# StorjOld/heartbeat

Hardware: AMD Instinct MI355X
Metric: GiB/s file bytes tagged (Swizzle encode, device-resident) at 1/2/4/8 GPUs (higher is better)
Workload: dtype u32

## Files before the change

heartbeat_amd/csrc/hb_args.hpp:

```cpp
#pragma once
#include "hb_lane.hpp"
#include "hb_digest_cache.hpp"

extern thread_local bool hb_load_only;

#ifndef HB_ENGINE_WG
#define HB_ENGINE_WG 1024
#endif
#define HB_ENGINE_WG_PER_CU 1
#ifndef HB_QUEUE_CHUNK
#define HB_QUEUE_CHUNK 256
#endif
#define HB_MAX_TRIES 2048u
#define HB_QSLOT 4
#define HB_SLOT_RETRY 7

#ifndef HB_RETRY_DIGEST
#define HB_RETRY_DIGEST 1
#endif
struct HbRetry {
    u64 blk;
    u32 flags;
    u32 pad_;
    u32 sr[4];
    u32 part[8];
#if HB_RETRY_DIGEST
    u32 dig[8];
#endif
};

#define HB_MFMA_MAX_S 2048u
#if defined(HB_MFMA_TOEPLITZ)
#define HB_MFMA_NT 2
#else
#define HB_MFMA_NT 1
#endif

template <int NL>
struct EncodeArgs {
    PrfParams<NL> prf;
    ModP<NL> mod;
    const unsigned char *data;
    u64 len;
    u64 nblocks;
    u64 block_base;
    unsigned char *tags;
    const u32 *alpha_mont;
    const u32 *t0;
// ... 225 lines not shown
```

heartbeat_amd/csrc/hb_kernels.hpp:

```cpp
#pragma once
#include <hip/hip_runtime.h>
#include "hb_args.hpp"
#include "hb_mac_src.hpp"

#define HB_LDS_WORDS (HB_TAB_BYTES / 4)

__device__ __forceinline__ void hb_fill_lds(u32 *lds, const u32 *t0) {
    for (u32 g = threadIdx.x; g < HB_LDS_WORDS / 4; g += blockDim.x) {
        const u32 off = g * 16u;
        const u32 e = (off >> 8) & 0xffu, t = ((off >> 16) << 1) | ((off >> 7) & 1u);
        u32 v = t0[e];
        if (t) v = (v << (8 * t)) | (v >> (32 - 8 * t));
        reinterpret_cast<uint4 *>(lds)[g] = make_uint4(v, v, v, v);
    }
    __syncthreads();
}

__device__ __forceinline__ LaneTab hb_lane_tab(const u32 *lds) {
    const u32 r4 = (threadIdx.x & 31u) * 4u;
    return LaneTab{(const char *)lds, {r4, 128u + r4, 0x10000u | r4, 0x10000u | (128u + r4)}};
}

__device__ __forceinline__ u32 hb_lane_id() { return threadIdx.x & 63u; }

// ... 22 lines not shown
        u64 base2 = 0, got2 = 0;
        if (avail < need && !exhausted) {
            u64 b = 0;
            if (hb_lane_id() == 0) b = atomicAdd(counter, (unsigned long long)chunk);
            b = hb_bcast64(b);
            if (b >= njobs) {
                exhausted = true;
            } else {
                base2 = b;
                got2 = njobs - b < chunk ? njobs - b : chunk;
            }
        }
        bool ok = false;
        if (want) {
            if ((u64)rank < avail) {
                job = next + rank;
                ok = true;
            } else if ((u64)rank - avail < got2) {
                job = base2 + ((u64)rank - avail);
                ok = true;
            }
        }
        if ((u64)need <= avail) {
            next += need;
        } else {
            const u64 used2 = (u64)need - avail < got2 ? (u64)need - avail : got2;
            next = base2 + used2;
            end = base2 + got2;
        }
        return ok;
    }
};

template <int MODE>
__device__ __forceinline__ void hb_prf_digest(u64 x, u32 dig[8]) {
    if (MODE != 0) hb_sha256_le32((u32)x, dig);
    else hb_sha256_decimal(x, dig);
}

template <int MODE, class H>
__device__ __forceinline__ auto hb_job_digest(const H &h, u64 job, u32 dig[8], int)
    -> decltype(h.digest(job, dig), void()) {
    if (!h.digest(job, dig)) hb_prf_digest<MODE>(h.x_of(job), dig);
}
template <int MODE, class H>
__device__ __forceinline__ void hb_job_digest(const H &h, u64 job, u32 dig[8], long) {
    hb_prf_digest<MODE>(h.x_of(job), dig);
}

template <class H>
__device__ __forceinline__ auto hb_resumed_tries(const H &, int) -> decltype(H::kResumedTries, u32()) {
    return H::kResumedTries;
}
template <class H>
__device__ __forceinline__ u32 hb_resumed_tries(const H &, long) { return 0u; }

template <int NL, int NR, class H, int MODE = 0>
__device__ __forceinline__ void hb_engine(H &h, const LaneTab &L, const PrfParams<NL> &P,
                                          u64 njobs, unsigned long long *queue, u64 chunk = HB_QUEUE_CHUNK) {
    HbPool pool{0, 0, njobs, queue, false, chunk};
    u64 job = 0;
    bool active = pool.take(__ballot(1), true, job);
    u32 dig[8], sr[4] = {0, 0, 0, 0}, out[NL];
    if (active) {
        h.init(job, sr);
        hb_job_digest<MODE>(h, job, dig, 0);
    }
    const u32 resumed = hb_resumed_tries(h, 0);
    u32 tries = 0, job_tries = resumed, failed = 0;
    while (__ballot(active)) {
        u32 ok;
        if constexpr (MODE == 1) ok = hb_cxx_try<NL, NR>(L, P, sr, dig, out);
        else if constexpr (MODE == 2) ok = hb_cxx_try_bytes<NL, NR>(L, P, sr, dig, out, job_tries);
        else ok = hb_prf_try<NL, NR>(L, P, sr, dig, out);
        tries += active ? 1u : 0u;
        job_tries += 1u;
        if (MODE != 0 && job_tries >= HB_CXX_MAX_TRIES) ok = 1;
        const bool acc = active && ok;
        if (acc) h.accept(job, out);
        const bool give_up = active && !ok && job_tries >= HB_MAX_TRIES;
        failed += give_up ? 1u : 0u;
        const bool next = acc || give_up;
        const u64 m = __ballot(next);
        if (m) {
            u64 nj = 0;
            const bool got = pool.take(m, next, nj);
            if (next) {
                active = got;
                job = nj;
                job_tries = resumed;
                if (got) {
                    h.init(job, sr);
                    hb_job_digest<MODE>(h, job, dig, 0);
                }
            }
        }
    }
    for (int off = 32; off > 0; off >>= 1) {
        tries += __shfl_xor(tries, off);
        failed += __shfl_xor(failed, off);
    }
    if (hb_lane_id() == 0 && tries) atomicAdd(queue + 1, (unsigned long long)tries);
    if (hb_lane_id() == 0 && failed) atomicAdd(queue + 2, (unsigned long long)failed);
}

#define HB_QP(a, b, c, d) ((a) | ((b) << 2) | ((c) << 4) | ((d) << 6))

template <int CTRL>
__device__ __forceinline__ u32 hb_qdpp(u32 x) {
    return (u32)__builtin_amdgcn_mov_dpp((int)x, CTRL, 0xf, 0xf, false);
}
__device__ __forceinline__ u64 hb_qbcast64(u64 v) {
    const u32 lo = hb_qdpp<HB_QP(0, 0, 0, 0)>((u32)v), hi = hb_qdpp<HB_QP(0, 0, 0, 0)>((u32)(v >> 32));
    return ((u64)hi << 32) | lo;
}

struct QuadLane {
    LaneTab L;
    u32 lbq;
// ... 68 lines not shown
        if (nw == 0) word &= (P.topmask << (24 - sh)) | (0xffffffu >> sh);
        HB_UNROLL
        for (int t = NL - 1; t > 0; --t) out[t] = hb_alignbit(out[t], out[t - 1], sh);
        out[0] = hb_alignbit(out[0], word << sh, sh);
    }
    u32 borrow = 0;
    HB_UNROLL
    for (int t = 0; t < NL; ++t) {
        u64 d = (u64)out[t] - (u64)P.R[t] - (u64)borrow;
        borrow = (u32)(d >> 63);
    }
    return borrow;
}

template <int NL, int NR, class H>
__device__ __forceinline__ void hb_engine_quad(H &h, const LaneTab &L, const PrfParams<NL> &P, u64 njobs,
                                               unsigned long long *queue, u64 chunk, u64 first = ~0ull,
                                               u64 end = ~0ull) {
    const QuadLane Q = hb_quad_lane(L);
    const u32 q = hb_lane_id() & 3u;
    const bool lead = q == 0;
    u32 rkq[NR + 1];
    HB_UNROLL
    for (int r = 0; r <= NR; ++r) {
        const u32 k0 = __builtin_amdgcn_readfirstlane(P.rk[4 * r]), k1 = __builtin_amdgcn_readfirstlane(P.rk[4 * r + 1]);
        const u32 k2 = __builtin_amdgcn_readfirstlane(P.rk[4 * r + 2]), k3 = __builtin_amdgcn_readfirstlane(P.rk[4 * r + 3]);
        rkq[r] = q == 0 ? k0 : q == 1 ? k1 : q == 2 ? k2 : k3;
    }
    u64 stop = njobs - first < 16 ? njobs : first + 16;
    if (stop > end) stop = end;
    HbPool pool = first == ~0ull ? HbPool{0, 0, njobs, queue, false, chunk}
                                 : HbPool{first, stop, njobs, queue, true, chunk};
    u64 job = 0;
    bool active = pool.take(__ballot(lead), lead, job);
    job = hb_qbcast64(job);
    active = hb_qdpp<HB_QP(0, 0, 0, 0)>(active ? 1u : 0u) != 0;
    u32 dig[8], s = 0, out[NL];
    if (active) hb_job_digest<0>(h, job, dig, 0);
    u32 tries = 0, job_tries = 0, failed = 0;
    while (__ballot(active)) {
        const u32 ok = hb_quad_prf_try<NL, NR>(Q, rkq, P, s, dig, out);
        tries += active && lead ? 1u : 0u;
        job_tries += 1u;
        const bool acc = active && ok;
        if (acc && lead) h.accept(job, out);
        const bool give_up = active && !ok && job_tries >= HB_MAX_TRIES;
        failed += give_up && lead ? 1u : 0u;
        if (give_up && lead) h.fail(job);
        const bool next = acc || give_up;
        const u64 m = __ballot(next && lead);
        if (m) {
            u64 nj = 0;
            bool got = pool.take(m, next && lead, nj);
            nj = hb_qbcast64(nj);
            got = hb_qdpp<HB_QP(0, 0, 0, 0)>(got ? 1u : 0u) != 0;
            if (next) {
                active = got;
                job = nj;
                job_tries = 0;
                if (got) {
                    s = 0;
                    hb_job_digest<0>(h, job, dig, 0);
                }
            }
        }
    }
    for (int off = 32; off > 0; off >>= 1) {
        tries += __shfl_xor(tries, off);
        failed += __shfl_xor(failed, off);
    }
    if (hb_lane_id() == 0 && tries) atomicAdd(queue + 1, (unsigned long long)tries);
    if (hb_lane_id() == 0 && failed) atomicAdd(queue + 2, (unsigned long long)failed);
}

#ifndef HB_RETRY_QUAD_TAIL
#define HB_RETRY_QUAD_TAIL 1
#endif
template <int NL, int NR, class H>
__device__ __forceinline__ void hb_engine_tail(H &h, const LaneTab &L, const PrfParams<NL> &P, u64 njobs,
                                               unsigned long long *queue, u64 chunk) {
    HbPool pool{0, 0, njobs, queue, false, chunk};
    u64 job = 0;
    bool active = pool.take(__ballot(1), true, job);
    u32 dig[8], sr[4] = {0, 0, 0, 0}, out[NL];
    if (active) {
        h.init(job, sr);
        hb_job_digest<0>(h, job, dig, 0);
    }
    const u32 resumed = hb_resumed_tries(h, 0);
    u32 tries = 0, job_tries = resumed, failed = 0;
    u64 am;
    while ((am = __ballot(active)) != 0) {
        if (pool.exhausted && pool.next >= pool.end && __popcll(am) <= 16) break;
        const u32 ok = hb_prf_try<NL, NR>(L, P, sr, dig, out);
        tries += active ? 1u : 0u;
        job_tries += 1u;
        const bool acc = active && ok;
        if (acc) h.accept(job, out);
        const bool give_up = active && !ok && job_tries >= HB_MAX_TRIES;
        failed += give_up ? 1u : 0u;
        const bool next = acc || give_up;
        const u64 m = __ballot(next);
        if (m) {
            u64 nj = 0;
            const bool got = pool.take(m, next, nj);
            if (next) {
                active = got;
                job = nj;
                job_tries = resumed;
                if (got) {
                    h.init(job, sr);
                    hb_job_digest<0>(h, job, dig, 0);
                }
            }
        }
    }
    if (am) {
        const u32 lane = hb_lane_id(), r = lane >> 2, q = lane & 3u;
        const bool qa = r < (u32)__popcll(am);
        u64 mm = am;
        for (u32 k = 0; k < r && mm; ++k) mm &= mm - 1;
        const int src = mm ? __builtin_ctzll(mm) : 0;
        const u64 qjob = ((u64)(u32)__shfl((int)(u32)(job >> 32), src) << 32) | (u32)__shfl((int)(u32)job, src);
        u32 qdig[8];
        HB_UNROLL
        for (int t = 0; t < 8; ++t) qdig[t] = (u32)__shfl((int)dig[t], src);
        const u32 w0 = (u32)__shfl((int)sr[0], src), w1 = (u32)__shfl((int)sr[1], src);
        const u32 w2 = (u32)__shfl((int)sr[2], src), w3 = (u32)__shfl((int)sr[3], src);
        u32 s = q == 0 ? w0 : q == 1 ? w1 : q == 2 ? w2 : w3;
        u32 jt = (u32)__shfl((int)job_tries, src);
        const QuadLane Q = hb_quad_lane(L);
        u32 rkq[NR + 1];
        HB_UNROLL
        for (int rr = 0; rr <= NR; ++rr) {
            const u32 k0 = __builtin_amdgcn_readfirstlane(P.rk[4 * rr]), k1 = __builtin_amdgcn_readfirstlane(P.rk[4 * rr + 1]);
            const u32 k2 = __builtin_amdgcn_readfirstlane(P.rk[4 * rr + 2]), k3 = __builtin_amdgcn_readfirstlane(P.rk[4 * rr + 3]);
            rkq[rr] = q == 0 ? k0 : q == 1 ? k1 : q == 2 ? k2 : k3;
        }
// ... 419 lines not shown
    v[NL] = T[NL] + (u32)c;
    hb_reduce_small<NL>(v, M, out);
}
#endif

template <int NL>
__device__ __forceinline__ uint4 *hb_dig_entry(const EncodeArgs<NL> &A, u64 blk) {
    return reinterpret_cast<uint4 *>(A.dig_tab + (A.block_base + blk - A.dig_lo) * 8);
}

template <int NL>
__device__ __forceinline__ void hb_dig_load(const EncodeArgs<NL> &A, u64 blk, u32 dig[8]) {
    const uint4 *e = hb_dig_entry<NL>(A, blk);
    const uint4 a = e[0], b = e[1];
    dig[0] = a.x; dig[1] = a.y; dig[2] = a.z; dig[3] = a.w;
    dig[4] = b.x; dig[5] = b.y; dig[6] = b.z; dig[7] = b.w;
}

template <int NL, bool DLOAD>
__device__ __forceinline__ void hb_first_digest(const EncodeArgs<NL> &A, u64 job, bool act, u32 dig[8]) {
    if constexpr (DLOAD) {
        hb_dig_load<NL>(A, job, dig);
        return;
    }
    hb_sha256_decimal(A.block_base + job, dig);
    if (A.dig_mode == HB_DIG_STORE && act) {
        uint4 *e = hb_dig_entry<NL>(A, job);
        e[0] = make_uint4(dig[0], dig[1], dig[2], dig[3]);
        e[1] = make_uint4(dig[4], dig[5], dig[6], dig[7]);
    }
}

template <int NL>
__device__ __forceinline__ void hb_list_early(const EncodeArgs<NL> &A, u64 job, u64 mask, const u32 dig[8],
                                              u64 &base) {
#if HB_RETRY_DIGEST
    u64 b = 0;
    if (hb_lane_id() == 0) b = atomicAdd(A.retry_count, (unsigned long long)__popcll(mask));
    base = hb_bcast64(b);
    if ((mask >> hb_lane_id()) & 1ull) {
        const u64 slot = base + hb_mbcnt(mask);
        if (slot < A.retry_cap) {
            HbRetry *e = A.retry + slot;
            *reinterpret_cast<uint4 *>(e) = make_uint4((u32)job, (u32)(job >> 32), 1u, 0u);
            *reinterpret_cast<uint4 *>(e->dig) = make_uint4(dig[0], dig[1], dig[2], dig[3]);
            *reinterpret_cast<uint4 *>(e->dig + 4) = make_uint4(dig[4], dig[5], dig[6], dig[7]);
        }
    }
#endif
}

template <int NL, int NR, int ALIGN, class H>
__device__ __forceinline__ void hb_first_finish(const EncodeArgs<NL> &A, const LaneTab &L, H &h, u64 job,
                                                bool active, u32 ok, u32 sr[4], u32 out[NL], u32 &tries,
                                                u32 &failed, u32 *T, bool tmine, u64 pre_base, u64 pre_mask) {
    tries += active ? 1u : 0u;
    const bool rejected = active && !ok;
    const bool pre = (pre_mask >> hb_lane_id()) & 1ull;
    const u64 rej = __ballot(rejected && !pre);
    bool listed = false;
    HbRetry *e = nullptr;
    if (pre) {
        const u64 slot = pre_base + hb_mbcnt(pre_mask);
        if (slot < A.retry_cap) {
            listed = true;
            e = A.retry + slot;
        }
    }
    if (rej) {
        u64 base = 0;
        if (hb_lane_id() == 0) base = atomicAdd(A.retry_count, (unsigned long long)__popcll(rej));
        base = hb_bcast64(base);
        if (rejected && !pre) {
            const u64 slot = base + hb_mbcnt(rej);
            if (slot < A.retry_cap) {
                listed = true;
                e = A.retry + slot;
                *reinterpret_cast<uint4 *>(e) = make_uint4((u32)job, (u32)(job >> 32), 0u, 0u);
            }
        }
    }
    if (listed) {
        *reinterpret_cast<uint4 *>(e->sr) = make_uint4(sr[0], sr[1], sr[2], sr[3]);
    } else if (rejected) {
        u32 dig[8];
        hb_sha256_decimal(A.block_base + job, dig);
        u32 n = 1;
        while (!ok && n < HB_MAX_TRIES) {
            ok = hb_prf_try<NL, NR>(L, A.prf, sr, dig, out);
            ++n;
            ++tries;
        }
        failed += ok ? 0u : 1u;
    }
    const bool done = active && ok;
#if defined(HB_EXP_NO_FINISH)
    if (done) hb_store_be<NL>(A.tags + job * (u64)A.tw, A.tw, T + 3);
    return;
#endif
    if constexpr (NL == 8) {
        if (A.mfma) {
            if (tmine && (done || listed)) {
                u32 F[NL], res[NL];
                HB_UNROLL
                for (int t = 0; t < NL; ++t) F[t] = done ? out[t] : 0u;
                hb_finish_T<NL>(T, F, A.mod, res);
                if (done) {
                    hb_store_tag<NL, ALIGN>(A.tags + job * (u64)A.tw, A.tw, res);
                } else {
                    *reinterpret_cast<uint4 *>(e->part) = make_uint4(res[0], res[1], res[2], res[3]);
                    *reinterpret_cast<uint4 *>(e->part + 4) = make_uint4(res[4], res[5], res[6], res[7]);
                }
                return;
            }
            if (listed) {
                const u32 zero[NL] = {0, 0, 0, 0, 0, 0, 0, 0};
                u32 part[NL];
                hb_block_tag<NL, ALIGN>(A.data, A.len, job, A.C, A.ss, A.S, A.alpha_mont, A.mod, zero, part);
                *reinterpret_cast<uint4 *>(e->part) = make_uint4(part[0], part[1], part[2], part[3]);
                *reinterpret_cast<uint4 *>(e->part + 4) = make_uint4(part[4], part[5], part[6], part[7]);
                return;
            }
        }
    }
    if (done) h.accept(job, out);
}

template <int NL, int NR, int ALIGN, bool DLOAD>
__device__ __forceinline__ void hb_encode_first_body(const EncodeArgs<NL> &A) {
    constexpr bool MF = NL == 8 && ALIGN == 16;
    constexpr u32 AFW = MF ? HB_MFMA_NT * HB_MFMA_LDS_S * 64u * 4u : 0u;
    __shared__ __attribute__((aligned(16))) u32 lds[HB_LDS_WORDS + AFW];
    const bool alds = MF && A.mfma && A.S <= HB_MFMA_LDS_S;
    if (alds) {
        const uint4 *src = reinterpret_cast<const uint4 *>(A.afrag);
        uint4 *dst = reinterpret_cast<uint4 *>(lds + HB_LDS_WORDS);
        for (u32 k = threadIdx.x; k < HB_MFMA_NT * A.S * 64u; k += blockDim.x) dst[k] = src[k];
    }
    hb_fill_lds(lds, A.t0);
    const LaneTab L = hb_lane_tab(lds);
    EncodeHandler<NL, ALIGN> h{A};
    HbPool pool{0, 0, A.nblocks, A.queue, false, hb_qchunk(A.qchunk)};
    u32 tries = 0, failed = 0;
    for (;;) {
        u64 job = 0;
        const bool act = pool.take(__ballot(1), true, job);
        if (!__ballot(act)) break;
        u32 T[2 * NL + 1];
        bool tmine = false;
#if defined(HB_EXP_NO_MFMA)
        for (int t = 0; t <= 2 * NL; ++t) T[t] = (u32)job + t;
        tmine = act && hb_block_full(A, job);
        if (0)
#endif
        if constexpr (MF) {
            const hb_i32x4 *afl_lds = reinterpret_cast<const hb_i32x4 *>(lds + HB_LDS_WORDS);
            const hb_i32x4 *afl_glb = reinterpret_cast<const hb_i32x4 *>(A.afrag);
#if !defined(HB_MFMA_TOEPLITZ)
            if (A.mfma == 3) {
                if (alds) tmine = hb_mfma16_block_acc<NL, true>(A, afl_lds, job, act, T);
                else tmine = hb_mfma16_block_acc<NL, false>(A, afl_glb, job, act, T);
            } else
#endif
            if (alds) tmine = hb_mfma_block_acc<NL, true>(A, afl_lds, job, act, T);
            else if (A.mfma) tmine = hb_mfma_block_acc<NL, false>(A, afl_glb, job, act, T);
        }
        u32 out[NL], sr[4], ok;
        u64 pre_base = 0, pre_mask = 0;
        {
            u32 dig[8];
            hb_first_digest<NL, DLOAD>(A, job, act, dig);
            hb_prf_prefix<NL>(A.pfx, A.o0, A.prf, dig[0], sr, out);
#if HB_RETRY_DIGEST
            pre_mask = __ballot(act && out[0] > A.rtop);
            if (pre_mask) hb_list_early<NL>(A, job, pre_mask, dig, pre_base);
#endif
            __builtin_amdgcn_s_setprio(HB_AES_PRIO);
            ok = hb_prf_try_from<NL, NR, 1>(L, A.prf, sr, dig, out);
            __builtin_amdgcn_s_setprio(0);
        }
        hb_first_finish<NL, NR, ALIGN>(A, L, h, job, act, ok, sr, out, tries, failed, T, tmine, pre_base,
                                       pre_mask);
    }
    for (int off = 32; off > 0; off >>= 1) {
        tries += __shfl_xor(tries, off);
        failed += __shfl_xor(failed, off);
    }
    if (hb_lane_id() == 0 && tries) atomicAdd(A.queue + 1, (unsigned long long)tries);
    if (hb_lane_id() == 0 && failed) atomicAdd(A.queue + 2, (unsigned long long)failed);
}

template <int NL, int NR, int ALIGN>
__global__ __launch_bounds__((HbEncWg<NL, ALIGN>::v), HbEncodeOcc<NL>::v) void hb_encode_first_kernel(EncodeArgs<NL> A) {
    hb_encode_first_body<NL, NR, ALIGN, false>(A);
}

template <int NL, int NR, int ALIGN>
__global__ __launch_bounds__((HbEncWg<NL, ALIGN>::v), HbEncodeOcc<NL>::v) void hb_encode_first_load_kernel(EncodeArgs<NL> A) {
    hb_encode_first_body<NL, NR, ALIGN, true>(A);
}

template <int NL, int ALIGN>
struct RetryHandler {
    static constexpr u32 kResumedTries = 1;
    const EncodeArgs<NL> &A;
    __device__ __forceinline__ u64 x_of(u64 job) const { return A.block_base + A.retry[job].blk; }
    __device__ __forceinline__ void init(u64 job, u32 sr[4]) const {
        const uint4 v = *reinterpret_cast<const uint4 *>(A.retry[job].sr);
        sr[0] = v.x; sr[1] = v.y; sr[2] = v.z; sr[3] = v.w;
    }
    __device__ __forceinline__ bool digest(u64 job, u32 dig[8]) const {
        const HbRetry &r = A.retry[job];
        if (A.dig_mode != HB_DIG_NONE) {
            hb_dig_load<NL>(A, r.blk, dig);
            return true;
        }
#if HB_RETRY_DIGEST
        if (!(r.flags & 1u)) return false;
        const uint4 a = *reinterpret_cast<const uint4 *>(r.dig), b = *reinterpret_cast<const uint4 *>(r.dig + 4);
        dig[0] = a.x; dig[1] = a.y; dig[2] = a.z; dig[3] = a.w;
        dig[4] = b.x; dig[5] = b.y; dig[6] = b.z; dig[7] = b.w;
        return true;
#else
        return false;
#endif
    }
    __device__ __forceinline__ void accept(u64 job, const u32 F[NL]) const {
        const u64 blk = A.retry[job].blk;
        if constexpr (ALIGN == 0) {
            hb_store_limbs<NL>(A.fout + blk * NL, F);
            return;
        } else {
        u32 tag[NL];
        if (NL == 8 && A.mfma) {
            u32 v[NL + 1];
            u64 c = 0;
            for (int t = 0; t < NL; ++t) {
                c += (u64)F[t] + A.retry[job].part[t < 8 ? t : 0];
// ... 889 lines not shown
```

heartbeat_amd/csrc/hb_runtime.cpp:

```cpp
#include <hip/hip_runtime.h>
#include <math.h>
#include <chrono>
#include <stdio.h>
#include <stdlib.h>
#include <string.h>
#include <condition_variable>
#include <exception>
#include <memory>
#include <mutex>
#include <string>
#include <atomic>
#include <thread>
#include <type_traits>
#include <vector>

#include "../../include/hbswizzle.h"
#include "hb_aes_host.hpp"
#include "hb_args.hpp"
#include "hb_wide_args.hpp"
#include "hb_vbatch_args.hpp"
#include "hb_pbatch_args.hpp"
#include "hb_cbatch_args.hpp"
#include "hb_cpv_args.hpp"
#include "hb_mixed_args.hpp"
#include "hb_cmixed_args.hpp"
#include "hb_emixed_args.hpp"
#include "hb_prime_args.hpp"
#include "hb_bignum_host.hpp"
#include "hb_batch_host.hpp"
#include "hb_mixed_host.hpp"
#include "hb_pv_host.hpp"
#include "hb_emixed_host.hpp"
#include "hb_prime_host.hpp"
#include "hb_merkle_host.hpp"
#include "hb_onehash_host.hpp"

using namespace hbhost;

template <int NL> hipError_t hb_launch_encode(const EncodeArgs<NL> &, int, int, int, int, hipStream_t);
template <int NL> hipError_t hb_launch_mac(const EncodeArgs<NL> &, int, hipStream_t);
template <int NL> hipError_t hb_launch_prf_pair(const Prf2Args<NL> &, int, int, hipStream_t);
hipError_t hb_launch_prefix(const PrefixArgs &, int, int, hipStream_t);
template <int NL> hipError_t hb_launch_prf(const PrfArgs<NL> &, int, int, int, hipStream_t);
template <int NL> hipError_t hb_launch_mont(const MontArgs<NL> &, hipStream_t);
template <int NL> hipError_t hb_launch_wsum(const WsumArgs<NL> &, int, int, hipStream_t);
template <int NL> hipError_t hb_launch_prove_prf(const ProveArgs<NL> &, int, int, int, int, hipStream_t);
template <int NL> hipError_t hb_launch_verify_fused(const VerifyArgs<NL> &, int, int, hipStream_t);
hipError_t hb_launch_fill(unsigned char *, u64, u64, hipStream_t);
hipError_t hb_launch_read(const void *, u64, u32 *, int, hipStream_t);
hipError_t hb_launch_merkle_offsets(const MerkleArgs &, int, hipStream_t);
hipError_t hb_launch_hmac(const MerkleArgs &, hipStream_t);
// ... 353 lines not shown
        for (int pass = 1; pass <= 3; ++pass) (void)hb_launch_encode<NL>(E, 14, 0, pass, 0, c->stream);
        (void)hb_launch_encode<NL>(EL, 14, 0, 1, 0, c->stream);
        WtabArgs<NL> WT;
        memset(&WT, 0, sizeof WT);
        (void)hb_launch_wtab<NL>(WT, c->stream);
        WmacArgs<NL> WM;
        memset(&WM, 0, sizeof WM);
        (void)hb_launch_wmac<NL>(WM, c->stream);
    }
    for (int align : {16, 1}) (void)hb_launch_mac<NL>(E, align, c->stream);
    Prf2Args<NL> P2;
    memset(&P2, 0, sizeof P2);
    (void)hb_launch_prf_pair<NL>(P2, 14, 0, c->stream);
    PrfArgs<NL> P;
    memset(&P, 0, sizeof P);
    for (int mode : {0, 3}) (void)hb_launch_prf<NL>(P, 14, mode, 0, c->stream);
    if constexpr (NL <= HB_FUSE_MAX_NL) {
        VerifyArgs<NL> VA;
        memset(&VA, 0, sizeof VA);
        (void)hb_launch_verify_fused<NL>(VA, 14, 0, c->stream);
    }
    MontArgs<NL> M;
    memset(&M, 0, sizeof M);
    (void)hb_launch_mont<NL>(M, c->stream);
    WsumArgs<NL> W;
    memset(&W, 0, sizeof W);
    for (int align : {16, 1}) (void)hb_launch_wsum<NL>(W, align, 0, c->stream);
    ProveArgs<NL> V;
    memset(&V, 0, sizeof V);
    (void)hb_launch_prove_prf<NL>(V, 14, 3, 3, 0, c->stream);
    (void)hb_launch_prove_prf<NL>(V, 14, 0, 0, 0, c->stream);
}

u64 retry_capacity(const hb_ctx *c, const uint8_t *p_be, size_t p_len, u64 nb) {
    size_t i = 0;
    while (i < p_len && p_be[i] == 0) ++i;
    u64 top = 0;
    size_t k = 0;
    for (; k < 8 && i + k < p_len; ++k) top = (top << 8) | p_be[i + k];
    const int rest = 8 * (int)(p_len - i - k);
    const double frac = ldexp((double)top, rest - bitlen_be(p_be, p_len));
    double q = 1.0 - frac;
    if (q < 0) q = 0;
    const double mean = q * (double)nb;
    double cap = mean + 8.0 * sqrt(mean) + 1024.0;
    if (const char *t = sw_env(c, "HB_TEST_RETRY_CAP")) cap = fmin(cap, atof(t));
    return cap >= (double)nb ? nb : (u64)cap;
}

int mfma_tables_begin(hb_ctx *c, u32 S) {
    const int NL = 8;
    if (c->h2d_pending) {
        HB_CHECK(hipEventSynchronize(c->ev_h2d), "H2D(afrag)");
        c->h2d_pending = false;
    }
    if (c->alpha_pending) {
        HB_CHECK(hipStreamSynchronize(c->stream), "D2H(alpha)");
        c->alpha_pending = false;
    }
    HB_CHECK(c->hscratch.ensure((size_t)S * NL * 4 + (size_t)HB_MFMA_NT * S * 64 * 16), "hipHostMalloc(scratch)");
#if !defined(HB_MFMA_TOEPLITZ) && !defined(HB_MAC_MONT)
    const void *asrc = c->alpha_raw.p;
#else
    const void *asrc = c->alpha_mont.p;
#endif
    HB_CHECK(hipMemcpyAsync(c->hscratch.p, asrc, (size_t)S * NL * 4, hipMemcpyDeviceToHost, c->stream), "D2H(alpha)");
    c->alpha_pending = true;
    HB_CHECK(hipEventRecord(c->ev_alpha, c->stream), "hipEventRecord");
    return 0;
}

int mfma_tables(hb_ctx *c, const Limbs &p, u32 S, u32 kz[17], int layout) {
    const int NL = 8;
    u32 *am = (u32 *)c->hscratch.p;
    int8_t *frag = (int8_t *)c->hscratch.p + (size_t)S * NL * 4;
    const size_t frag_bytes = (size_t)HB_MFMA_NT * S * 64 * 16;
    HB_CHECK(hipEventSynchronize(c->ev_alpha), "alpha PRF");
    c->alpha_pending = false;
    auto src_of = [&](u32 slot, int h, int e, u32 &j, int &k) {
        if (layout == 2) {
// ... 524 lines not shown
            if (int rc2 = wide_prep<NL>(c, p, pi, w, WT)) return rc2;
            const size_t fbytes = (size_t)WT.nslices * WT.Mt * 64 * 16;
            HB_CHECK(c->wtab.ensure(fbytes + (size_t)(NL + 1) * 4 + 16), "hipMalloc(wide table)");
            WT.mod = A.mod;
            WT.S = S;
            WT.alpha_mont = (const u32 *)c->alpha_mont.p;
            WT.afrag = (int8_t *)c->wtab.p;
            WT.kz = (u32 *)((uint8_t *)c->wtab.p + fbytes);
            WT.status = (unsigned int *)(WT.kz + NL + 1);
            f_in_tags = !small && pi.tw == 4u * NL && (uintptr_t)dtags % 16 == 0;
            if (!f_in_tags) HB_CHECK(c->vals.ensure((size_t)launch_blocks * NL * 4), "hipMalloc(F)");
            mark("wide tables");
        }
    }
    const bool side = !small && wide && !sw_env(c, "HB_WIDE_SYNC_ALPHA");
    hipStream_t ast = side ? c->side : c->stream;
    if (side) {
        HB_CHECK(hipEventRecord(c->ev_side0, c->stream), "hipEventRecord");
        HB_CHECK(hipStreamWaitEvent(c->side, c->ev_side0, 0), "hipStreamWaitEvent");
    }
    if (!small) {
        rc = run_prf<NL>(c, a_key, key_len, p_be, p_len, nullptr, 0, S, (u32 *)c->alpha_raw.p, 1, cxx ? 1 : 0,
                         nullptr, ast);
        if (rc) return rc;
        mark("alpha PRF");
        rc = run_mont<NL>(c, p, (const u32 *)c->alpha_raw.p, (u32 *)c->alpha_mont.p, S, ast);
        if (rc) return rc;
        mark("alpha PRF + Montgomery");
    }
    if (two_pass) {
        A.retry_cap = retry_capacity(c, p_be, p_len, launch_blocks);
        HB_CHECK(c->retry.ensure((size_t)(A.retry_cap ? A.retry_cap : 1) * sizeof(HbRetry)), "hipMalloc(retry)");
        A.retry = (HbRetry *)c->retry.p;
        A.retry_count = q0 + 3;
        mark("retry list");
    }
    if (!data_dev) {
        HB_CHECK(c->data[0].ensure((size_t)(cb * C)), "hipMalloc(staging)");
        HB_CHECK(c->data[1].ensure((size_t)(cb * C)), "hipMalloc(staging)");
    }
    c->dig_next_set = false;
    c->dig_last_mode = HB_DIG_NONE;
    if (two_pass) {
        A.dig_mode = c->dig_last_mode = dig_prepare(c, block_base, nblocks);
        A.dig_tab = (u32 *)c->dig.p;
        A.dig_lo = c->dig_alloc.lo;
        if (A.dig_mode != HB_DIG_NONE) A.rtop = 0xffffffffu;
        mark("digest table");
    }
    if (two_pass && !cxx) {
        HB_CHECK(c->pfx.ensure(HB_PFX_BYTES), "hipMalloc(prefix)");
        A.pfx = (const unsigned char *)c->pfx.p;
        AesKey k;
        aes_expand(f_key, key_len, k);
        uint8_t zero[16] = {0}, o[16];
        aes_encrypt_block(k, zero, o);
        A.o0 = o[0];
        mark("prefix image buffer");
    }
    if (mf_layout) {
        rc = mfma_tables_begin(c, S);
        if (rc) return rc;
    }
    c->last_launches = 0;
    c->ph_valid = false;
    float ms_total = 0.f;
    HB_CHECK(hipEventRecord(c->k0, c->stream), "hipEventRecord");
// ... 108 lines not shown
                alpha_todo = false;
            }
            const EngineShape es = quad_engine(c, nb + F2.S);
            F.qchunk = es.chunk;
            F.place = placed ? 1u : 0u;
            if (!placed) {
                HB_CHECK(hipMemsetAsync(q0, 0, sizeof(unsigned long long), c->stream), "hipMemsetAsync");
                HB_CHECK(hb_launch_prf<NL>(F, nr, 3, (int)c->num_cus, c->stream), "hb_prf_kernel launch");
            } else if (F2.S) {
                HB_CHECK(hb_launch_prf_pair<NL>(F2, nr, es.grid, c->stream), "hb_prf_pair_kernel launch");
            } else {
                HB_CHECK(hb_launch_prf<NL>(F, nr, 3, es.grid, c->stream), "hb_prf_kernel launch");
            }
            c->last_launches++;
            if (wide) {
                rc = wide_table();
                if (!rc) rc = wide_mac(d, dlen, nb, tg, (const u32 *)c->vals.p, align);
                return rc;
            }
            HB_CHECK(hb_launch_mac<NL>(A, align, c->stream), "hb_mac_kernel launch");
            c->last_launches++;
            return 0;
        }
        HB_CHECK(hipMemsetAsync(q0, 0, sizeof(unsigned long long), c->stream), "hipMemsetAsync");
        if (!two_pass) {
            A.queue = q0;
            if (wide) A.fout = f_in_tags ? (u32 *)tg : (u32 *)c->vals.p;
            HB_CHECK(hb_launch_encode<NL>(A, nr, wide ? 0 : align, cxx ? 3 : 0, engine_grid(c, nb), c->stream),
                     "hb_encode_kernel launch");
            c->last_launches++;
            if (wide) return wide_mac(d, dlen, nb, tg, A.fout, align);
            return 0;
        }
        HB_CHECK(hipMemsetAsync(q0 + 3, 0, sizeof(unsigned long long), c->stream), "hipMemsetAsync");
        A.queue = q0;
        if (data_dev) HB_CHECK(hipEventRecord(c->ph[0], c->stream), "hipEventRecord");
        const int palign = wide ? 0 : align;
        if (wide) A.fout = f_in_tags ? (u32 *)tg : (u32 *)c->vals.p;
        HB_CHECK(hb_launch_encode<NL>(A, nr, palign, 1, engine_grid(c, nb), c->stream),
                 "hb_encode_first_kernel launch");
        if (data_dev) HB_CHECK(hipEventRecord(c->ph[1], c->stream), "hipEventRecord");
        HB_CHECK(hipMemsetAsync(q7, 0, sizeof(unsigned long long), c->stream), "hipMemsetAsync");
        A.queue = q7;
        HB_CHECK(hb_launch_encode<NL>(A, nr, palign, 2, engine_grid(c, A.retry_cap), c->stream),
                 "hb_encode_retry_kernel launch");
        if (data_dev) HB_CHECK(hipEventRecord(c->ph[2], c->stream), "hipEventRecord");
        c->ph_valid = data_dev;
        c->last_launches += 2;
        if (wide) return wide_mac(d, dlen, nb, tg, A.fout, align);
        return 0;
    };

    if (data_dev) {
        rc = launch(data, len, nblocks, block_base, dtags);
        if (rc) return rc;
        HB_CHECK(hipEventRecord(c->k1, c->stream), "hipEventRecord");
        if (flags & HB_ASYNC) {
            c->pending = true;
            c->pend_q0 = q0;
            c->pend_q7 = q7;
            return 0;
        }
        HB_CHECK(hipEventSynchronize(c->k1), "encode");
        HB_CHECK(hipEventElapsedTime(&ms_total, c->k0, c->k1), "hipEventElapsedTime");
        mark("kernels");
    } else {
        HB_CHECK(c->data[0].ensure((size_t)(cb * C)), "hipMalloc(staging)");
// ... 1972 lines not shown
    auto bad = [&](hipError_t err, const char *what) {
        g_create_error = std::string(what) + ": " + hipGetErrorString(err);
        hb_ctx_destroy(c);
        return HB_EHIP;
    };
    if ((e = hipSetDevice(device)) != hipSuccess) return bad(e, "hipSetDevice");
    hipDeviceProp_t prop;
    if ((e = hipGetDeviceProperties(&prop, device)) != hipSuccess) return bad(e, "hipGetDeviceProperties");
    if (!strstr(prop.gcnArchName, "gfx950")) {
        g_create_error = std::string("libhbswizzle is built for gfx950 (MI355X); device is ") + prop.gcnArchName;
        hb_ctx_destroy(c);
        return HB_EUNSUPPORTED;
    }
    c->num_cus = prop.multiProcessorCount;
    if ((e = hipStreamCreateWithFlags(&c->stream, hipStreamNonBlocking)) != hipSuccess) return bad(e, "hipStreamCreate");
    c->own_stream = c->stream;
    if ((e = hipStreamCreateWithFlags(&c->copy, hipStreamNonBlocking)) != hipSuccess) return bad(e, "hipStreamCreate");
    if ((e = hipStreamCreateWithFlags(&c->side, hipStreamNonBlocking)) != hipSuccess) return bad(e, "hipStreamCreate");
    if ((e = hipEventCreateWithFlags(&c->ev_side0, hipEventDisableTiming)) != hipSuccess) return bad(e, "hipEventCreate");
    if ((e = hipEventCreateWithFlags(&c->ev_side1, hipEventDisableTiming)) != hipSuccess) return bad(e, "hipEventCreate");
    if ((e = hipEventCreate(&c->k0)) != hipSuccess) return bad(e, "hipEventCreate");
    if ((e = hipEventCreate(&c->k1)) != hipSuccess) return bad(e, "hipEventCreate");
    for (int k = 0; k < 3; ++k)
        if ((e = hipEventCreate(&c->ph[k])) != hipSuccess) return bad(e, "hipEventCreate");
    for (int b = 0; b < 2; ++b) {
        if ((e = hipEventCreateWithFlags(&c->copied[b], hipEventDisableTiming)) != hipSuccess) return bad(e, "hipEventCreate");
        if ((e = hipEventCreateWithFlags(&c->done[b], hipEventDisableTiming)) != hipSuccess) return bad(e, "hipEventCreate");
    }
    if ((e = hipEventCreateWithFlags(&c->ev_alpha, hipEventDisableTiming)) != hipSuccess) return bad(e, "hipEventCreate");
    if ((e = hipEventCreateWithFlags(&c->ev_h2d, hipEventDisableTiming)) != hipSuccess) return bad(e, "hipEventCreate");
    if ((e = hipMalloc(&c->t0, 256 * sizeof(u32))) != hipSuccess) return bad(e, "hipMalloc");
    if ((e = hipMemcpy(c->t0, aes_tables().t0, 256 * sizeof(u32), hipMemcpyHostToDevice)) != hipSuccess)
        return bad(e, "hipMemcpy");
    if ((e = hipMalloc(&c->queue, 16 * HB_QSLOT * sizeof(unsigned long long))) != hipSuccess) return bad(e, "hipMalloc");
    if ((e = hipMemset(c->queue, 0, 16 * HB_QSLOT * sizeof(unsigned long long))) != hipSuccess) return bad(e, "hipMemset");
    if ((e = c->hscratch.ensure(64u << 10)) != hipSuccess) return bad(e, "hipHostMalloc");
    *out = c;
    return HB_OK;
}

void hb_ctx_destroy(hb_ctx *c) {
    if (!c) return;
    (void)hipSetDevice(c->device);
    settle(c);
    if (c->stream) (void)hipStreamSynchronize(c->stream);
    if (c->copy) (void)hipStreamSynchronize(c->copy);
    if (c->side) (void)hipStreamSynchronize(c->side);
    DevBuf *bufs[] = {&c->alpha_raw, &c->alpha_mont, &c->xs, &c->vals, &c->vals2, &c->wts, &c->idx,
                      &c->partials, &c->sums, &c->data[0], &c->data[1], &c->tags, &c->blen, &c->gtags,
                      &c->pfx, &c->retry, &c->ctl, &c->afrag, &c->mseeds, &c->moffs, &c->mdig, &c->gdev,
                      &c->facc, &c->gup, &c->wpw, &c->wtab, &c->dig, &c->bdev, &c->pr_src, &c->pr_bases,
                      &c->pr_jobs, &c->pr_pass, &c->pr_q, &c->pr_win, &c->pr_surv, &c->pr_cnt,
                      &c->mk_files, &c->mk_seeds, &c->mk_offs, &c->mk_blobs, &c->mk_nodes, &c->mk_data,
                      &c->mk_gather, &c->oh_files, &c->oh_jobs, &c->oh_seeds, &c->oh_resp, &c->oh_data,
                      &c->oh_gather, &c->oh_draw, &c->oh_states};
    for (DevBuf *b : bufs) b->release();
    if (c->hres) (void)hipHostFree(c->hres);
    c->gstage[0].release();
    c->gstage[1].release();
    c->hscratch.release();
    c->bhost.release();
    c->mk_out.release();
    c->oh_out.release();
    c->oh_dout.release();
    if (c->t0) (void)hipFree(c->t0);
    if (c->queue) (void)hipFree(c->queue);
    if (c->k0) (void)hipEventDestroy(c->k0);
    if (c->k1) (void)hipEventDestroy(c->k1);
// ... 1616 lines not shown
```

Measured before the change: 1154.

## Reserve retry-list slots in per-wave slabs instead of per-wave atomics

Each wave now claims retry-list slots in slabs of 64 through one global atomic and hands them out locally. Before, it did an atomicAdd on the shared retry counter every time some lanes were rejected. Unused slab tails are filled with null sentinel entries, and the retry engine skips those entries when it takes jobs. The retry capacity is enlarged by the per-wave slack, and the counter moves to its own padded word in the queue buffer. This cuts contention on a hot global atomic, at the cost of larger retry buffers and extra null-skipping loops in the retry kernel.

```diff
diff --git a/heartbeat_amd/csrc/hb_args.hpp b/heartbeat_amd/csrc/hb_args.hpp
--- a/heartbeat_amd/csrc/hb_args.hpp
+++ b/heartbeat_amd/csrc/hb_args.hpp
@@ -14,6 +14,13 @@
 #define HB_MAX_TRIES 2048u
 #define HB_QSLOT 4
 #define HB_SLOT_RETRY 7
+#define HB_QUEUE_WORDS (16 * HB_QSLOT + 16)
+#define HB_RETRY_COUNT_WORD (16 * HB_QSLOT)
+#ifndef HB_RETRY_SLAB
+#define HB_RETRY_SLAB 64
+#endif
+static_assert(HB_RETRY_SLAB >= 64, "a slab must cover one request of a whole wave");
+#define HB_RETRY_NULL (~0ull)
 
 #ifndef HB_RETRY_DIGEST
 #define HB_RETRY_DIGEST 1
diff --git a/heartbeat_amd/csrc/hb_kernels.hpp b/heartbeat_amd/csrc/hb_kernels.hpp
--- a/heartbeat_amd/csrc/hb_kernels.hpp
+++ b/heartbeat_amd/csrc/hb_kernels.hpp
@@ -78,6 +78,46 @@
     }
 };
 
+#define HB_NO_SLOT 0xffffffffu
+struct HbGrant {
+    u32 b0, b1, n;
+    __device__ __forceinline__ u32 slot(u32 rank) const {
+        const u32 n0 = n & 0xffu, n1 = n >> 8;
+        if (rank < n0) return b0 + rank;
+        if (rank - n0 < n1) return b1 + (rank - n0);
+        return HB_NO_SLOT;
+    }
+};
+
+struct HbSlab {
+    u32 next, end;
+
+    __device__ __forceinline__ HbGrant reserve(unsigned long long *counter, u32 need, u64 cap) {
+        const u32 avail = end - next;
+        HbGrant g{next, 0, need};
+        if (need <= avail) {
+            next += need;
+            return g;
+        }
+        u32 got2 = 0;
+        if (next != HB_NO_SLOT) {
+            u64 b = 0;
+            if (hb_lane_id() == 0) b = atomicAdd(counter, (unsigned long long)HB_RETRY_SLAB);
+            b = hb_bcast64(b);
+            if (b < cap) {
+                g.b1 = (u32)b;
+                got2 = cap - b < (u64)HB_RETRY_SLAB ? (u32)(cap - b) : (u32)HB_RETRY_SLAB;
+            }
+        }
+        const u32 n1 = need - avail < got2 ? need - avail : got2;
+        g.n = avail | (n1 << 8);
+        next = g.b1 + n1;
+        end = g.b1 + got2;
+        if (got2 == 0) next = end = HB_NO_SLOT;
+        return g;
+    }
+};
+
 template <int MODE>
 __device__ __forceinline__ void hb_prf_digest(u64 x, u32 dig[8]) {
     if (MODE != 0) hb_sha256_le32((u32)x, dig);
@@ -100,13 +140,34 @@
 }
 template <class H>
 __device__ __forceinline__ u32 hb_resumed_tries(const H &, long) { return 0u; }
+
+template <class H>
+constexpr auto hb_has_null_jobs(int) -> decltype(&H::null_job, bool()) { return true; }
+template <class H>
+constexpr bool hb_has_null_jobs(long) { return false; }
+
+template <class H>
+__device__ __forceinline__ bool hb_deal(HbPool &pool, const H &h, u64 mask, bool want, u64 &job) {
+    if constexpr (!hb_has_null_jobs<H>(0)) {
+        return pool.take(mask, want, job);
+    } else {
+        bool got = false;
+        for (;;) {
+            const bool g = pool.take(mask, want, job);
+            if (want) got = g;
+            want = want && g && h.null_job(job);
+            mask = __ballot(want);
+            if (!mask) return got;
+        }
+    }
+}
 
 template <int NL, int NR, class H, int MODE = 0>
 __device__ __forceinline__ void hb_engine(H &h, const LaneTab &L, const PrfParams<NL> &P,
                                           u64 njobs, unsigned long long *queue, u64 chunk = HB_QUEUE_CHUNK) {
     HbPool pool{0, 0, njobs, queue, false, chunk};
     u64 job = 0;
-    bool active = pool.take(__ballot(1), true, job);
+    bool active = hb_deal(pool, h, __ballot(1), true, job);
     u32 dig[8], sr[4] = {0, 0, 0, 0}, out[NL];
     if (active) {
         h.init(job, sr);
@@ -130,7 +191,7 @@
         const u64 m = __ballot(next);
         if (m) {
             u64 nj = 0;
-            const bool got = pool.take(m, next, nj);
+            const bool got = hb_deal(pool, h, m, next, nj);
             if (next) {
                 active = got;
                 job = nj;
@@ -265,7 +326,7 @@
     HbPool pool = first == ~0ull ? HbPool{0, 0, njobs, queue, false, chunk}
                                  : HbPool{first, stop, njobs, queue, true, chunk};
     u64 job = 0;
-    bool active = pool.take(__ballot(lead), lead, job);
+    bool active = hb_deal(pool, h, __ballot(lead), lead, job);
     job = hb_qbcast64(job);
     active = hb_qdpp<HB_QP(0, 0, 0, 0)>(active ? 1u : 0u) != 0;
     u32 dig[8], s = 0, out[NL];
@@ -284,7 +345,7 @@
         const u64 m = __ballot(next && lead);
         if (m) {
             u64 nj = 0;
-            bool got = pool.take(m, next && lead, nj);
+            bool got = hb_deal(pool, h, m, next && lead, nj);
             nj = hb_qbcast64(nj);
             got = hb_qdpp<HB_QP(0, 0, 0, 0)>(got ? 1u : 0u) != 0;
             if (next) {
@@ -314,7 +375,7 @@
                                                unsigned long long *queue, u64 chunk) {
     HbPool pool{0, 0, njobs, queue, false, chunk};
     u64 job = 0;
-    bool active = pool.take(__ballot(1), true, job);
+    bool active = hb_deal(pool, h, __ballot(1), true, job);
     u32 dig[8], sr[4] = {0, 0, 0, 0}, out[NL];
     if (active) {
         h.init(job, sr);
@@ -336,7 +397,7 @@
         const u64 m = __ballot(next);
         if (m) {
             u64 nj = 0;
-            const bool got = pool.take(m, next, nj);
+            const bool got = hb_deal(pool, h, m, next, nj);
             if (next) {
                 active = got;
                 job = nj;
@@ -822,15 +883,14 @@
 }
 
 template <int NL>
-__device__ __forceinline__ void hb_list_early(const EncodeArgs<NL> &A, u64 job, u64 mask, const u32 dig[8],
-                                              u64 &base) {
+__device__ __forceinline__ HbGrant hb_list_early(const EncodeArgs<NL> &A, HbSlab &slab, u64 job, u64 mask,
+                                                 const u32 dig[8]) {
+    HbGrant g{0, 0, 0};
 #if HB_RETRY_DIGEST
-    u64 b = 0;
-    if (hb_lane_id() == 0) b = atomicAdd(A.retry_count, (unsigned long long)__popcll(mask));
-    base = hb_bcast64(b);
+    g = slab.reserve(A.retry_count, (u32)__popcll(mask), A.retry_cap);
     if ((mask >> hb_lane_id()) & 1ull) {
-        const u64 slot = base + hb_mbcnt(mask);
-        if (slot < A.retry_cap) {
+        const u32 slot = g.slot(hb_mbcnt(mask));
+        if (slot != HB_NO_SLOT) {
             HbRetry *e = A.retry + slot;
             *reinterpret_cast<uint4 *>(e) = make_uint4((u32)job, (u32)(job >> 32), 1u, 0u);
             *reinterpret_cast<uint4 *>(e->dig) = make_uint4(dig[0], dig[1], dig[2], dig[3]);
@@ -838,50 +898,63 @@
         }
     }
 #endif
+    return g;
+}
+
+template <int NL>
+__device__ __forceinline__ HbRetry *hb_first_list(const EncodeArgs<NL> &A, const HbGrant &g, u64 job,
+                                                  bool rejected, const HbGrant &pre_g, u64 pre_mask, u64 rej,
+                                                  bool &listed) {
+    const bool pre = (pre_mask >> hb_lane_id()) & 1ull;
+    HbRetry *e = nullptr;
+    if (pre) {
+        const u32 slot = pre_g.slot(hb_mbcnt(pre_mask));
+        if (slot != HB_NO_SLOT) {
+            listed = true;
+            e = A.retry + slot;
+        }
+    }
+    if (rejected && !pre) {
+        const u32 slot = g.slot(hb_mbcnt(rej));
+        if (slot != HB_NO_SLOT) {
+            listed = true;
+            e = A.retry + slot;
+            *reinterpret_cast<uint4 *>(e) = make_uint4((u32)job, (u32)(job >> 32), 0u, 0u);
+        }
+    }
+    return e;
+}
+
+template <int NL, int NR>
+__device__ __forceinline__ void hb_first_in_place(const EncodeArgs<NL> &A, const LaneTab &L, u64 job, u32 &ok,
+                                                  u32 sr[4], u32 out[NL], u32 &tries, u32 &failed) {
+    u32 dig[8];
+    hb_sha256_decimal(A.block_base + job, dig);
+    u32 n = 1;
+    while (!ok && n < HB_MAX_TRIES) {
+        ok = hb_prf_try<NL, NR>(L, A.prf, sr, dig, out);
+        ++n;
+        ++tries;
+    }
+    failed += ok ? 0u : 1u;
 }
 
 template <int NL, int NR, int ALIGN, class H>
-__device__ __forceinline__ void hb_first_finish(const EncodeArgs<NL> &A, const LaneTab &L, H &h, u64 job,
-                                                bool active, u32 ok, u32 sr[4], u32 out[NL], u32 &tries,
-                                                u32 &failed, u32 *T, bool tmine, u64 pre_base, u64 pre_mask) {
+__device__ __forceinline__ void hb_first_finish(const EncodeArgs<NL> &A, const LaneTab &L, H &h, HbSlab &slab,
+                                                u64 job, bool active, u32 ok, u32 sr[4], u32 out[NL], u32 &tries,
+                                                u32 &failed, u32 *T, bool tmine, const HbGrant &pre_g,
+                                                u64 pre_mask) {
     tries += active ? 1u : 0u;
     const bool rejected = active && !ok;
-    const bool pre = (pre_mask >> hb_lane_id()) & 1ull;
-    const u64 rej = __ballot(rejected && !pre);
+    const u64 rej = __ballot(rejected && !((pre_mask >> hb_lane_id()) & 1ull));
+    HbGrant g{0, 0, 0};
+    if (rej) g = slab.reserve(A.retry_count, (u32)__popcll(rej), A.retry_cap);
     bool listed = false;
-    HbRetry *e = nullptr;
-    if (pre) {
-        const u64 slot = pre_base + hb_mbcnt(pre_mask);
-        if (slot < A.retry_cap) {
-            listed = true;
-            e = A.retry + slot;
-        }
-    }
-    if (rej) {
-        u64 base = 0;
-        if (hb_lane_id() == 0) base = atomicAdd(A.retry_count, (unsigned long long)__popcll(rej));
-        base = hb_bcast64(base);
-        if (rejected && !pre) {
-            const u64 slot = base + hb_mbcnt(rej);
-            if (slot < A.retry_cap) {
-                listed = true;
-                e = A.retry + slot;
-                *reinterpret_cast<uint4 *>(e) = make_uint4((u32)job, (u32)(job >> 32), 0u, 0u);
-            }
-        }
-    }
+    HbRetry *e = hb_first_list<NL>(A, g, job, rejected, pre_g, pre_mask, rej, listed);
     if (listed) {
         *reinterpret_cast<uint4 *>(e->sr) = make_uint4(sr[0], sr[1], sr[2], sr[3]);
     } else if (rejected) {
-        u32 dig[8];
-        hb_sha256_decimal(A.block_base + job, dig);
-        u32 n = 1;
-        while (!ok && n < HB_MAX_TRIES) {
-            ok = hb_prf_try<NL, NR>(L, A.prf, sr, dig, out);
-            ++n;
-            ++tries;
-        }
-        failed += ok ? 0u : 1u;
+        hb_first_in_place<NL, NR>(A, L, job, ok, sr, out, tries, failed);
     }
     const bool done = active && ok;
 #if defined(HB_EXP_NO_FINISH)
@@ -931,6 +1004,7 @@
     const LaneTab L = hb_lane_tab(lds);
     EncodeHandler<NL, ALIGN> h{A};
     HbPool pool{0, 0, A.nblocks, A.queue, false, hb_qchunk(A.qchunk)};
+    HbSlab slab{0, 0};
     u32 tries = 0, failed = 0;
     for (;;) {
         u64 job = 0;
@@ -956,21 +1030,26 @@
             else if (A.mfma) tmine = hb_mfma_block_acc<NL, false>(A, afl_glb, job, act, T);
         }
         u32 out[NL], sr[4], ok;
-        u64 pre_base = 0, pre_mask = 0;
+        u64 pre_mask = 0;
+        HbGrant pre_g{0, 0, 0};
         {
             u32 dig[8];
             hb_first_digest<NL, DLOAD>(A, job, act, dig);
             hb_prf_prefix<NL>(A.pfx, A.o0, A.prf, dig[0], sr, out);
 #if HB_RETRY_DIGEST
             pre_mask = __ballot(act && out[0] > A.rtop);
-            if (pre_mask) hb_list_early<NL>(A, job, pre_mask, dig, pre_base);
+            if (pre_mask) pre_g = hb_list_early<NL>(A, slab, job, pre_mask, dig);
 #endif
             __builtin_amdgcn_s_setprio(HB_AES_PRIO);
             ok = hb_prf_try_from<NL, NR, 1>(L, A.prf, sr, dig, out);
             __builtin_amdgcn_s_setprio(0);
         }
-        hb_first_finish<NL, NR, ALIGN>(A, L, h, job, act, ok, sr, out, tries, failed, T, tmine, pre_base,
+        hb_first_finish<NL, NR, ALIGN>(A, L, h, slab, job, act, ok, sr, out, tries, failed, T, tmine, pre_g,
                                        pre_mask);
+    }
+    if (hb_lane_id() < slab.end - slab.next) {
+        const u64 nul = HB_RETRY_NULL;
+        *reinterpret_cast<uint4 *>(A.retry + slab.next + hb_lane_id()) = make_uint4((u32)nul, (u32)(nul >> 32), 0u, 0u);
     }
     for (int off = 32; off > 0; off >>= 1) {
         tries += __shfl_xor(tries, off);
@@ -994,6 +1073,9 @@
 struct RetryHandler {
     static constexpr u32 kResumedTries = 1;
     const EncodeArgs<NL> &A;
+    __device__ __forceinline__ bool null_job(u64 job) const {
+        return (u32)(A.retry[job].blk >> 32) == (u32)(HB_RETRY_NULL >> 32);
+    }
     __device__ __forceinline__ u64 x_of(u64 job) const { return A.block_base + A.retry[job].blk; }
     __device__ __forceinline__ void init(u64 job, u32 sr[4]) const {
         const uint4 v = *reinterpret_cast<const uint4 *>(A.retry[job].sr);
diff --git a/heartbeat_amd/csrc/hb_retry_cap.hpp b/heartbeat_amd/csrc/hb_retry_cap.hpp
--- /dev/null
+++ b/heartbeat_amd/csrc/hb_retry_cap.hpp
@@ -0,0 +1,21 @@
+#pragma once
+#include <cmath>
+#include <cstdint>
+
+#define HB_RETRY_MAX_SLOTS 0xfffffffeull
+inline uint64_t hb_retry_slots(double q, uint64_t nb, uint64_t waves, uint64_t slab, double test_cap) {
+    if (nb == 0) return 0;
+    if (!(q > 0.0)) q = 0.0;
+    if (q > 1.0) q = 1.0;
+    const double mean = q * (double)nb;
+    const double want = mean + 8.0 * std::sqrt(mean) + 1024.0;
+    const uint64_t evals = want >= (double)nb ? nb : (uint64_t)want;
+    if (waves > 0xffffffffull) waves = 0xffffffffull;
+    if (slab < 1) slab = 1;
+    if (slab > 0x10000ull) slab = 0x10000ull;
+    const uint64_t slack = waves * (slab - 1);
+    uint64_t cap = evals + slack < evals ? ~0ull : evals + slack;
+    if (cap > HB_RETRY_MAX_SLOTS) cap = HB_RETRY_MAX_SLOTS;
+    if (test_cap >= 0.0 && test_cap < (double)cap) cap = (uint64_t)test_cap;
+    return cap;
+}
diff --git a/heartbeat_amd/csrc/hb_runtime.cpp b/heartbeat_amd/csrc/hb_runtime.cpp
--- a/heartbeat_amd/csrc/hb_runtime.cpp
+++ b/heartbeat_amd/csrc/hb_runtime.cpp
@@ -17,6 +17,7 @@
 #include "../../include/hbswizzle.h"
 #include "hb_aes_host.hpp"
 #include "hb_args.hpp"
+#include "hb_retry_cap.hpp"
 #include "hb_wide_args.hpp"
 #include "hb_vbatch_args.hpp"
 #include "hb_pbatch_args.hpp"
@@ -436,7 +437,7 @@
     (void)hb_launch_prove_prf<NL>(V, 14, 0, 0, 0, c->stream);
 }
 
-u64 retry_capacity(const hb_ctx *c, const uint8_t *p_be, size_t p_len, u64 nb) {
+u64 retry_capacity(hb_ctx *c, const uint8_t *p_be, size_t p_len, u64 nb) {
     size_t i = 0;
     while (i < p_len && p_be[i] == 0) ++i;
     u64 top = 0;
@@ -444,12 +445,9 @@
     for (; k < 8 && i + k < p_len; ++k) top = (top << 8) | p_be[i + k];
     const int rest = 8 * (int)(p_len - i - k);
     const double frac = ldexp((double)top, rest - bitlen_be(p_be, p_len));
-    double q = 1.0 - frac;
-    if (q < 0) q = 0;
-    const double mean = q * (double)nb;
-    double cap = mean + 8.0 * sqrt(mean) + 1024.0;
-    if (const char *t = sw_env(c, "HB_TEST_RETRY_CAP")) cap = fmin(cap, atof(t));
-    return cap >= (double)nb ? nb : (u64)cap;
+    const u64 waves = (u64)engine_grid(c, nb) * (HB_ENGINE_WG / 64);
+    const char *t = sw_env(c, "HB_TEST_RETRY_CAP");
+    return hb_retry_slots(1.0 - frac, nb, waves, HB_RETRY_SLAB, t ? atof(t) : -1.0);
 }
 
 int mfma_tables_begin(hb_ctx *c, u32 S) {
@@ -1040,7 +1038,7 @@
         A.retry_cap = retry_capacity(c, p_be, p_len, launch_blocks);
         HB_CHECK(c->retry.ensure((size_t)(A.retry_cap ? A.retry_cap : 1) * sizeof(HbRetry)), "hipMalloc(retry)");
         A.retry = (HbRetry *)c->retry.p;
-        A.retry_count = q0 + 3;
+        A.retry_count = c->queue + HB_RETRY_COUNT_WORD;
         mark("retry list");
     }
     if (!data_dev) {
@@ -1215,7 +1213,7 @@
             if (wide) return wide_mac(d, dlen, nb, tg, A.fout, align);
             return 0;
         }
-        HB_CHECK(hipMemsetAsync(q0 + 3, 0, sizeof(unsigned long long), c->stream), "hipMemsetAsync");
+        HB_CHECK(hipMemsetAsync(A.retry_count, 0, sizeof(unsigned long long), c->stream), "hipMemsetAsync");
         A.queue = q0;
         if (data_dev) HB_CHECK(hipEventRecord(c->ph[0], c->stream), "hipEventRecord");
         const int palign = wide ? 0 : align;
@@ -3254,8 +3252,8 @@
     if ((e = hipMalloc(&c->t0, 256 * sizeof(u32))) != hipSuccess) return bad(e, "hipMalloc");
     if ((e = hipMemcpy(c->t0, aes_tables().t0, 256 * sizeof(u32), hipMemcpyHostToDevice)) != hipSuccess)
         return bad(e, "hipMemcpy");
-    if ((e = hipMalloc(&c->queue, 16 * HB_QSLOT * sizeof(unsigned long long))) != hipSuccess) return bad(e, "hipMalloc");
-    if ((e = hipMemset(c->queue, 0, 16 * HB_QSLOT * sizeof(unsigned long long))) != hipSuccess) return bad(e, "hipMemset");
+    if ((e = hipMalloc(&c->queue, HB_QUEUE_WORDS * sizeof(unsigned long long))) != hipSuccess) return bad(e, "hipMalloc");
+    if ((e = hipMemset(c->queue, 0, HB_QUEUE_WORDS * sizeof(unsigned long long))) != hipSuccess) return bad(e, "hipMemset");
     if ((e = c->hscratch.ensure(64u << 10)) != hipSuccess) return bad(e, "hipHostMalloc");
     *out = c;
     return HB_OK;
```

Result: no change. 1155 (median of 3 runs) (+0.1%).
